# bcsefercik/markerless-robot-camera-calibration

Hardware: AMD Instinct MI355X
Metric: point-cloud frames/sec at 200k pts/frame (higher is better)
Workload: dtype f32

## Files before the change

### markerless-robot-camera-calibration_amd/csrc/sv_conv.hip

```cpp
#include <stdarg.h>
#include <stdio.h>
#include <stdlib.h>
#include <vector>

#include "sv_conv_params.h"

namespace sv {

static thread_local char g_last_instance[128] = "";
static thread_local double g_want_scale_override = -1.0;
static thread_local double g_tail_override = -1.0;
void note_instance(const char* fmt, ...) {
  va_list ap;
  va_start(ap, fmt);
  vsnprintf(g_last_instance, sizeof(g_last_instance), fmt, ap);
  va_end(ap);
}
#ifndef SV_CONV_WANT_SCALE_DEFAULT
#define SV_CONV_WANT_SCALE_DEFAULT 0.3
#endif
#ifndef SV_CONV_TAIL_DEFAULT
#define SV_CONV_TAIL_DEFAULT 0.15
#endif
constexpr int chunk_for(int tm, int waves_n) {
  if (waves_n == 1) return tm <= 64 ? 128 : 64;
  if (waves_n == 2) return tm <= 32 ? 128 : (tm <= 64 ? 64 : 32);
  return tm <= 16 ? 128 : (tm <= 32 ? 64 : 32);
}

constexpr int fused_offsets(int cpo) { return cpo == 0 ? 1 : (cpo < 8 ? 27 : (128 / cpo > 0 ? 128 / cpo : 1)); }
constexpr int lds_row_stride(int kc) {
  for (int sa = kc + 2;; ++sa)
    if (sa % 64 == 34 || (sa % 4 == 0 && (sa / 4) % 2 == 1)) return sa;
}

template <int TM_, int WAVES_N, int NT, int CPO = 0>
struct ConvCfg {
  static constexpr int WAVES_M = 4 / WAVES_N;
  static constexpr int MR = TM_ / WAVES_M / 16;
  static constexpr int TN = WAVES_N * NT * 16;
  static constexpr int GK = fused_offsets(CPO);
  static constexpr int KC = CPO ? (GK * CPO + 3) / 4 * 4 : chunk_for(TM_, WAVES_N);
  static constexpr int SA = lds_row_stride(KC);
  static constexpr int PFD_RAW = MR * NT >= 6 ? 1 : (8 + MR * NT - 1) / (MR * NT);
  static constexpr int PFD = PFD_RAW > KC / 4 ? KC / 4 : PFD_RAW;
  static constexpr bool USE_FULL = (MR * NT == 1) || (TM_ == 32 && WAVES_N == 4 && NT == 3) || (TM_ == 16 && NT == 3);
  static constexpr int F4_PER_ROW = KC / 4;
  static constexpr int ROWS_PER_PASS = 256 / F4_PER_ROW;
  static constexpr int A_F4 = (TM_ + ROWS_PER_PASS - 1) / ROWS_PER_PASS;
  static_assert(MR >= 1, "tile too small for the wave layout");
  static constexpr size_t lds_bytes(int K) { return (size_t)(2 * TM_ * SA + K * TM_) * sizeof(float); }
};

template <int TM_, int WAVES_N, int NT, bool FAST, int CPO = 0, bool RING = false, bool FULL = false>
__device__ __forceinline__ void conv_tile_body(const ConvParams& p, const int bidx, const int tile_base) {
  static_assert(FAST || !FULL, "FULL is a refinement of the FAST form");
  using Cfg = ConvCfg<TM_, WAVES_N, NT, CPO>;
  constexpr int MR = Cfg::MR, TN = Cfg::TN, A_F4 = Cfg::A_F4, KC = Cfg::KC, SA = Cfg::SA, GK = Cfg::GK;
  constexpr int PFD = RING ? Cfg::PFD : 1;
  constexpr int ROWS_PER_PASS = Cfg::ROWS_PER_PASS;
  constexpr int SUBS = TM_ / 16;
  extern __shared__ __attribute__((aligned(16))) float lds[];
  float* As = lds;
  int* idx_s = (int*)(lds + 2 * TM_ * SA);

  const int tid = threadIdx.x;
  const int lane = tid & 63;
  const int wid = __builtin_amdgcn_readfirstlane(tid >> 6);
  const int wm = wid / WAVES_N, wn = wid % WAVES_N;
  unsigned long long trace_t0 = 0, trace_t_loop = 0, trace_t_epi = 0;
  int trace_steps = 0;
  if (p.trace) trace_t0 = wall_clock64();
  const int ny = (p.Cout + TN - 1) / TN;
  constexpr int SUB_PER_PLAN_TILE = PLAN_TILE / TM_;
  const int t_lin = bidx / ny;
  const int t128 = tile_base + t_lin / SUB_PER_PLAN_TILE;
  const int p128 = p.tile_order ? p.tile_order[t128] : ((int)(p.Vpad / PLAN_TILE) - 1 - t128);
  const int tile = p128 * SUB_PER_PLAN_TILE + (t_lin % SUB_PER_PLAN_TILE);
  const int n0 = (bidx % ny) * TN;
  const int64_t row0 = (int64_t)tile * TM_;
  const int li = lane & 15, lq = lane >> 4;
  const int K = p.K, Cin = p.Cin, Cout = p.Cout;
  const int col0 = n0 + wn * NT * 16 + NT * li;
  const bool cols_full = col0 + NT <= Cout;

  f32x4 acc[MR][NT];
#pragma unroll
  for (int s = 0; s < MR; ++s)
#pragma unroll
    for (int n = 0; n < NT; ++n) acc[s][n] = (f32x4){0.f, 0.f, 0.f, 0.f};

  if (p.acc_init) {
    if constexpr (FAST) {
      const __amdgpu_buffer_rsrc_t rsrc_acc = __builtin_amdgcn_make_buffer_rsrc((void*)p.acc_init, 0, (int)p.acc_bytes, 0x00020000);
      int o_acc[MR][4];
      load_perm_rows<MR>(p, row0 + wm * MR * 16, lane >> 4, o_acc);
#pragma unroll
      for (int s = 0; s < MR; ++s)
#pragma unroll
        for (int reg = 0; reg < 4; ++reg) {
          const auto v = buffer_load_floats<NT>(
              rsrc_acc, o_acc[s][reg] >= 0 ? (uint32_t)o_acc[s][reg] * (uint32_t)(p.acc_ld * 4) + (uint32_t)col0 * 4u : BUF_ABSENT, 0u);
#pragma unroll
          for (int n = 0; n < NT; ++n) acc[s][n][reg] = v[n];
        }
    } else {
#pragma unroll
      for (int s = 0; s < MR; ++s)
#pragma unroll
        for (int reg = 0; reg < 4; ++reg) {
          const int64_t r = row0 + wm * MR * 16 + s * 16 + (lane >> 4) * 4 + reg;
          const int64_t o = p.perm ? (int64_t)p.perm[r] : (r < p.V_out ? r : -1);
#pragma unroll
          for (int n = 0; n < NT; ++n) acc[s][n][reg] = (o >= 0 && col0 + n < Cout) ? p.acc_init[o * p.acc_ld + col0 + n] : 0.0f;
        }
    }
  }
  uint32_t dense_mask = (1u << SUBS) - 1u;
  if (p.submask == nullptr) {
    const int64_t rem = p.V_out - row0;
    const int nsub = rem >= TM_ ? SUBS : (int)((rem + 15) / 16);
    dense_mask = (1u << nsub) - 1u;
  }
  if constexpr (FAST) {
    constexpr int STAGE_IT = (32 * TM_ + 255) / 256;
    int n_st[STAGE_IT];
#pragma unroll
    for (int it = 0; it < STAGE_IT; ++it) {
      const int e = tid + 256 * it;
      const int k = e / TM_, r = e % TM_;
      n_st[it] = -1;
      if (e < K * TM_) {
        if (p.nbr_s)
          n_st[it] = p.nbr_s[(int64_t)k * p.Vpad + row0 + r];
        else
          n_st[it] = (row0 + r < p.V_out) ? (int)(row0 + r) : -1;
      }
    }
#pragma unroll
    for (int it = 0; it < STAGE_IT; ++it) {
      const int e = tid + 256 * it;
      if (e < K * TM_) idx_s[e] = (int)(n_st[it] >= 0 ? (uint32_t)n_st[it] * (uint32_t)(p.in_ld * 4) : BUF_ABSENT);
    }
  } else {
    for (int e = tid; e < K * TM_; e += 256) {
      const int k = e / TM_, r = e - k * TM_;
      int n;
      if (p.nbr_s)
        n = p.nbr_s[(int64_t)k * p.Vpad + row0 + r];
      else
        n = (row0 + r < p.V_out) ? (int)(row0 + r) : -1;
      idx_s[e] = n;
    }
  }
  const __amdgpu_buffer_rsrc_t rsrc_in = __builtin_amdgcn_make_buffer_rsrc((void*)p.in, 0, (int)p.in_bytes, 0x00020000);
  const __amdgpu_buffer_rsrc_t rsrc_w = __builtin_amdgcn_make_buffer_rsrc((void*)p.W, 0, (int)p.w_bytes, 0x00020000);

  const int64_t sm_word = row0 / PLAN_TILE;
  const int sm_shift = (int)((row0 % PLAN_TILE) / 16);
  uint32_t my_sm = 0;
  if (lane < K) my_sm = p.submask ? ((p.submask[sm_word * K + lane] >> sm_shift) & ((1u << SUBS) - 1u)) : dense_mask;
  const uint32_t amask = (uint32_t)__ballot(my_sm != 0);
  auto fused_mask = [&](int k0) -> uint32_t {
    uint32_t m = 0;
#pragma unroll
    for (int g = 0; g < GK; ++g) m |= (uint32_t)__builtin_amdgcn_readlane((int)my_sm, min(k0 + g, 31));
    return m;
  };
  int k_n, c_n = 0;
  uint32_t sm_n = 0;
  bool have_n;
  if (CPO) {
    k_n = 0;
    while (k_n < K && (sm_n = fused_mask(k_n)) == 0) k_n += GK;
    have_n = k_n < K;
  } else {
    k_n = amask ? __builtin_ctz(amask) : K;
    sm_n = amask ? (uint32_t)__builtin_amdgcn_readlane((int)my_sm, k_n) : 0u;
    have_n = amask != 0;
  }
  auto advance = [&]() {
    if (CPO) {
      k_n += GK;
      while (k_n < K && (sm_n = fused_mask(k_n)) == 0) k_n += GK;
      have_n = k_n < K;
      return;
    }
    c_n += KC;
    if (c_n >= Cin) {
      c_n = 0;
      const uint32_t rest = amask & ~((2u << k_n) - 1u);
      have_n = rest != 0;
      k_n = have_n ? __builtin_ctz(rest) : K;
      sm_n = (uint32_t)__builtin_amdgcn_readlane((int)my_sm, have_n ? k_n : 0);
    }
  };

  float4 ra[A_F4];
  const int a_cc = (tid % Cfg::F4_PER_ROW) * 4;
  const int a_r = tid / Cfg::F4_PER_ROW;

  const uint32_t col_bytes = (uint32_t)a_cc * 4u;
  const int cin_rem = Cin % KC;
  const uint32_t col_last = (cin_rem == 0 || a_cc < cin_rem) ? col_bytes : 0u - (uint32_t)(Cin - cin_rem) * 4u;
  auto load_a = [&](int k, int c0, uint32_t sm) {
#pragma unroll
    for (int j = 0; j < A_F4; ++j) {
      const int r = a_r + ROWS_PER_PASS * j;
      if (FAST) {
        const int rr = (A_F4 * ROWS_PER_PASS > TM_) ? min(r, TM_ - 1) : r;
        if (CPO) {
          const int kk = k + a_cc / (CPO ? CPO : 1);
          uint32_t off = (uint32_t)idx_s[min(kk, K - 1) * TM_ + rr];
          if (kk >= K) off = BUF_ABSENT;
          const f32x4 v = buffer_load_floats<4>(rsrc_in, off + (uint32_t)(a_cc % (CPO ? CPO : 1)) * 4u, 0u);
          ra[j] = make_float4(v[0], v[1], v[2], v[3]);
        } else {
          const uint32_t off = (uint32_t)idx_s[k * TM_ + rr];
          const uint32_t cb = (!FULL && c0 + KC > Cin) ? col_last : col_bytes;
          const f32x4 v = buffer_load_floats<4>(rsrc_in, off + cb, (uint32_t)c0 * 4u);
          ra[j] = make_float4(v[0], v[1], v[2], v[3]);
        }
        (void)sm;
      } else if (CPO) {
        float e[4] = {0.f, 0.f, 0.f, 0.f};
        if (r < TM_ && ((sm >> (r >> 4)) & 1u)) {
#pragma unroll
          for (int q = 0; q < 4; ++q) {
            const int i = a_cc + q, kk = k + i / (CPO ? CPO : 1), c = i % (CPO ? CPO : 1);
            if (i < GK * CPO && kk < K) {
              const int n = idx_s[kk * TM_ + r];
              if (n >= 0) e[q] = p.in[(int64_t)n * p.in_ld + c];
            }
          }
        }
        ra[j] = make_float4(e[0], e[1], e[2], e[3]);
      } else {
        float4 v = make_float4(0.f, 0.f, 0.f, 0.f);
        if (r < TM_ && ((sm >> (r >> 4)) & 1u)) {
          const int n = idx_s[k * TM_ + r];
          const int c = c0 + a_cc;
          if (n >= 0) {
            const float* src = p.in + (int64_t)n * p.in_ld + c;
            if (p.vec_a) {
              if (c < Cin) v = *(const float4*)src;
            } else {
              if (c + 0 < Cin) v.x = src[0];
              if (c + 1 < Cin) v.y = src[1];
              if (c + 2 < Cin) v.z = src[2];
              if (c + 3 < Cin) v.w = src[3];
            }
          }
        }
        ra[j] = v;
      }
    }
  };
  auto store_a = [&](float* dstbuf, uint32_t sm) {
#pragma unroll
    for (int j = 0; j < A_F4; ++j) {
      const int r = a_r + ROWS_PER_PASS * j;
      if (r < TM_ && (FAST || ((sm >> (r >> 4)) & 1u))) {
        float2* dst = (float2*)(dstbuf + r * SA + a_cc);
        dst[0] = make_float2(ra[j].x, ra[j].y);
        dst[1] = make_float2(ra[j].z, ra[j].w);
      }
    }
  };

  typedef float bvec_t __attribute__((ext_vector_type(NT)));
  typedef float bvec_load_t __attribute__((ext_vector_type(NT), aligned(4)));
  bvec_t b[KC / 4];
  const int b_off = lq * Cout + col0;
  const uint32_t b_off_bytes = (uint32_t)b_off * 4u;
  auto step_weights = [&](int k, int c0) -> const float* { return p.W + ((int64_t)k * Cin + c0) * Cout; };
  auto cols_of = [&](int k, int c0) { return CPO ? min(GK, K - k) * CPO : min(KC, Cin - c0); };
  auto ksteps_of = [&](int k, int c0) { return (cols_of(k, c0) + 3) >> 2; };
  auto load_b = [&](const float* wstep, int k, int c0, int ksteps_valid, int ks, bvec_t& dst) {
    if (FAST) {
      const uint32_t row = (uint32_t)(k * Cin + c0 + (ks < ksteps_valid ? 4 * ks : 0));
      dst = buffer_load_floats<NT>(rsrc_w, b_off_bytes, row * (uint32_t)Cout * 4u);
      (void)wstep;
    } else {
      const int i = 4 * ks + lq;
      const float* src = p.W + ((int64_t)k * Cin + c0 + i) * Cout + col0;
      const bool row_ok = i < cols_of(k, c0);
#pragma unroll
      for (int n = 0; n < NT; ++n) dst[n] = (row_ok && col0 + n < Cout) ? src[n] : 0.0f;
    }
  };

  __syncthreads();
  if (have_n) {
    int k_c = k_n, c_c = c_n;
    uint32_t sm_c = sm_n;
    load_a(k_c, c_c, sm_c);
#pragma unroll
    for (int ks = 0; ks < KC / 4; ++ks) load_b(step_weights(k_c, c_c), k_c, c_c, ksteps_of(k_c, c_c), ks, b[ks]);
    store_a(As, sm_c);
    advance();
    int k_x = k_n, c_x = c_n;
    uint32_t sm_x = sm_n;
    bool have_x = have_n;
    __syncthreads();
    int buf = 0;
    if (p.trace) trace_t_loop = wall_clock64();

    auto step = [&]() -> bool {
      if (FAST || have_x) load_a(have_x ? k_x : 0, have_x ? c_x : 0, have_x ? sm_x : 0u);
      const float* a_base = As + buf * (TM_ * SA) + (wm * MR * 16 + li) * SA + lq;
      const uint32_t smw = (sm_c >> (wm * MR)) & ((1u << MR) - 1u);
      const int ksteps = ksteps_of(k_c, c_c);
      const int kb = have_x ? k_x : 0;
      const int cb = have_x ? c_x : 0;
      const float* wnext = step_weights(kb, cb);
      const int ksteps_next = ksteps_of(kb, cb);
      {
        auto reload_b = [&](int ks) {
          if (FULL) {
            b[ks] = buffer_load_floats<NT>(rsrc_w, b_off_bytes, (uint32_t)(kb * Cin + cb + 4 * ks) * (uint32_t)Cout * 4u);
          } else if (FAST || have_x) {
            load_b(wnext, kb, cb, ksteps_next, ks, b[ks]);
          }
        };
        auto mfma_row = [&](int ks, const float (&a)[MR]) {
#pragma unroll
          for (int s = 0; s < MR; ++s) {
            if ((MR == 1 && Cfg::WAVES_M == 1) || ((smw >> s) & 1u)) {
#pragma unroll
              for (int n = 0; n < NT; ++n)
                acc[s][n] = __builtin_amdgcn_mfma_f32_16x16x4f32(a[s], b[ks][n], acc[s][n], 0, 0, 0);
            }
          }
        };
        if constexpr (PFD == 1) {
          float a_cur[MR];
#pragma unroll
          for (int s = 0; s < MR; ++s) a_cur[s] = a_base[s * 16 * SA];
#pragma unroll
          for (int ks = 0; ks < KC / 4; ++ks) {
            if (FULL || ks < ksteps) {
              float a_nx[MR];
              if (ks + 1 < KC / 4) {
#pragma unroll
                for (int s = 0; s < MR; ++s) a_nx[s] = a_base[s * 16 * SA + (ks + 1) * 4];
                if (FULL) __builtin_amdgcn_sched_barrier(0);
              }
              mfma_row(ks, a_cur);
              if (ks + 1 < KC / 4) {
#pragma unroll
                for (int s = 0; s < MR; ++s) a_cur[s] = a_nx[s];
              }
            }
            reload_b(ks);
            if (FULL) __builtin_amdgcn_sched_barrier(0);
          }
        } else {
          float a_ring[PFD + 1][MR];
#pragma unroll
          for (int d = 0; d < PFD; ++d)
#pragma unroll
            for (int s = 0; s < MR; ++s) a_ring[d][s] = a_base[s * 16 * SA + d * 4];
#pragma unroll
          for (int ks = 0; ks < KC / 4; ++ks) {
            if (FULL || ks < ksteps) {
              if (ks + PFD < KC / 4) {
#pragma unroll
                for (int s = 0; s < MR; ++s)
                  a_ring[(ks + PFD) % (PFD + 1)][s] = a_base[s * 16 * SA + (ks + PFD) * 4];
                if (FULL) __builtin_amdgcn_sched_barrier(0);
              }
              mfma_row(ks, a_ring[ks % (PFD + 1)]);
            }
            reload_b(ks);
            if (FULL) __builtin_amdgcn_sched_barrier(0);
          }
        }
      }
      ++trace_steps;
      if (!have_x) return false;
      store_a(As + (buf ^ 1) * (TM_ * SA), sm_x);
      k_c = k_x;
      c_c = c_x;
      sm_c = sm_x;
      advance();
      k_x = k_n;
      c_x = c_n;
      sm_x = sm_n;
      have_x = have_n;
      __syncthreads();
      buf ^= 1;
      return true;
    };
    while (step()) {
    }
  }

  if (p.trace) trace_t_epi = wall_clock64();
  float sc[NT], sh[NT];
#pragma unroll
  for (int n = 0; n < NT; ++n) {
    const bool ok = col0 + n < Cout;
    sc[n] = (p.scale && ok) ? p.scale[col0 + n] : 1.0f;
    sh[n] = (p.shift && ok) ? p.shift[col0 + n] : 0.0f;
  }
  if constexpr (FAST) {
    epilogue_buffered<MR, NT>(p, acc, row0 + wm * MR * 16, lq, col0);
  } else
#pragma unroll
  for (int s = 0; s < MR; ++s) {
#pragma unroll
    for (int reg = 0; reg < 4; ++reg) {
      const int64_t r = row0 + wm * MR * 16 + s * 16 + lq * 4 + reg;
      int64_t o;
      if (p.perm)
        o = p.perm[r];
      else
        o = (r < p.V_out) ? r : -1;
      if (o < 0) continue;
      float y[NT];
#pragma unroll
      for (int n = 0; n < NT; ++n) {
        float v = acc[s][n][reg];
        if (p.scale)
          v = __builtin_fmaf(v, sc[n], sh[n]);
        else if (p.shift)
          v = v + sh[n];
        y[n] = v;
      }
      if (p.residual) {
        const float* res = p.residual + o * p.res_ld + col0;
#pragma unroll
        for (int n = 0; n < NT; ++n)
          if (col0 + n < Cout) y[n] = y[n] + res[n];
      }
      float* dst = p.out + o * p.out_ld + col0;
#pragma unroll
      for (int n = 0; n < NT; ++n) {
        float v = y[n];
        if (p.act == SV_ACT_RELU)
          v = v < 0.f ? 0.f : v;
        else if (p.act == SV_ACT_LEAKY_RELU)
          v = v > 0.f ? v : v * p.slope;
        if (col0 + n < Cout) dst[n] = v;
      }
    }
  }
  if (p.trace && tid == 0) {
    unsigned long long* t = p.trace + (size_t)blockIdx.x * 4;
    t[0] = trace_t0;
    t[1] = wall_clock64();
    t[2] = ((unsigned long long)__builtin_amdgcn_s_getreg((31 << 11) | 20) << 32) |
           (unsigned)__builtin_amdgcn_s_getreg((31 << 11) | 4);
    const unsigned long long pro = trace_t_loop ? ((trace_t_loop - trace_t0) >> 4) & 0xffffull : 0ull;
    const unsigned long long epi = ((t[1] - trace_t_epi) >> 4) & 0xffffull;
    t[3] = (unsigned long long)(unsigned)trace_steps | (pro << 32) | (epi << 48);
  }
}

template <int TM_, int WAVES_N, int NT, bool FAST, int CPO = 0, bool RING = false, bool FULL = false>
__global__ __launch_bounds__(256) void conv_fwd_kernel(ConvParams p) {
  conv_tile_body<TM_, WAVES_N, NT, FAST, CPO, RING, FULL>(p, (int)blockIdx.x, 0);
}

template <int TM_, int TAIL_TM, int WAVES_N, int NT, bool FAST>
__global__ __launch_bounds__(256) void conv_fwd_dual_kernel(ConvParams p) {
  if ((int)blockIdx.x < p.main_blocks)
    conv_tile_body<TM_, WAVES_N, NT, FAST>(p, (int)blockIdx.x, 0);
  else
    conv_tile_body<TAIL_TM, WAVES_N, NT, FAST>(p, (int)blockIdx.x - p.main_blocks, p.main_tiles128);
}

template <class Launch>
static int launch_traced(ConvParams& q, unsigned grid, int tm, int wn, int nt, hipStream_t stream, Launch&& launch) {
  static const char* trace_path = getenv("SV_CONV_TRACE");
  q.trace = nullptr;
  if (trace_path) SV_HIP(hipMalloc((void**)&q.trace, (size_t)grid * 4 * sizeof(unsigned long long)));
  launch();
  SV_LAUNCH_CHECK();
  if (q.trace) {
    std::vector<unsigned long long> host((size_t)grid * 4);
    SV_HIP(hipStreamSynchronize(stream));
    SV_HIP(hipMemcpy(host.data(), q.trace, host.size() * sizeof(unsigned long long), hipMemcpyDeviceToHost));
    SV_HIP(hipFree(q.trace));
    if (FILE* f = fopen(trace_path, "ab")) {
      const long long hdr[8] = {0x5356545243ll, (long long)grid, tm, wn, nt, q.ny, q.K, q.Cin};
      fwrite(hdr, sizeof(hdr), 1, f);
      fwrite(host.data(), sizeof(unsigned long long), host.size(), f);
      fclose(f);
    }
  }
  return SV_OK;
}

template <int TM_, int WAVES_N, int NT, int CPO = 0>
static int launch_conv(const ConvParams& p, hipStream_t stream) {
  using Cfg = ConvCfg<TM_, WAVES_N, NT, CPO>;
  ConvParams q = p;
  q.ntiles = (int)(p.Vpad / TM_);
  q.ny = (p.Cout + Cfg::TN - 1) / Cfg::TN;
  dim3 grid((unsigned)(q.ntiles * q.ny));
  const bool fast = p.vec_a && p.buf_ok && (p.Cout % Cfg::TN == 0);
  const bool ring = Cfg::PFD > 1 && grid.x <= 1024;
  constexpr bool F = (CPO % 4 == 0);
  const size_t lds = Cfg::lds_bytes(p.K);
  const bool full = Cfg::USE_FULL && (CPO ? (p.K % Cfg::GK == 0) : (p.Cin % Cfg::KC == 0));
  const int rc = launch_traced(q, grid.x, TM_, WAVES_N, NT, stream, [&] {
    if (F && fast && full) {
      if (ring)
        hipLaunchKernelGGL((conv_fwd_kernel<TM_, WAVES_N, NT, F, CPO, (Cfg::PFD > 1), (F && Cfg::USE_FULL)>), grid, dim3(256), lds, stream, q);
      else
        hipLaunchKernelGGL((conv_fwd_kernel<TM_, WAVES_N, NT, F, CPO, false, (F && Cfg::USE_FULL)>), grid, dim3(256), lds, stream, q);
    } else if (F && fast) {
      if (ring)
        hipLaunchKernelGGL((conv_fwd_kernel<TM_, WAVES_N, NT, F, CPO, (Cfg::PFD > 1)>), grid, dim3(256), lds, stream, q);
      else
        hipLaunchKernelGGL((conv_fwd_kernel<TM_, WAVES_N, NT, F, CPO, false>), grid, dim3(256), lds, stream, q);
    } else {
      if (ring)
        hipLaunchKernelGGL((conv_fwd_kernel<TM_, WAVES_N, NT, false, CPO, (Cfg::PFD > 1)>), grid, dim3(256), lds, stream, q);
      else
        hipLaunchKernelGGL((conv_fwd_kernel<TM_, WAVES_N, NT, false, CPO, false>), grid, dim3(256), lds, stream, q);
    }
  });
  if (rc != SV_OK) return rc;
  {
    const bool f = F && fast;
    if (CPO)
      note_instance("conv_fwd_kernel<%d, %d, %d, fused %d>|fast=%d,ring=%d,full=%d", TM_, WAVES_N, NT, CPO, (int)f, (int)ring,
                    (int)(f && full));
    else
      note_instance("conv_fwd_kernel<%d, %d, %d>|fast=%d,ring=%d,full=%d", TM_, WAVES_N, NT, (int)f, (int)ring, (int)(f && full));
  }
  return SV_OK;
}

template <int TM_, int TAIL_TM, int WAVES_N, int NT>
static int launch_conv_dual(const ConvParams& p, hipStream_t stream, double tail_fraction) {
  using Main = ConvCfg<TM_, WAVES_N, NT, 0>;
  using Tail = ConvCfg<TAIL_TM, WAVES_N, NT, 0>;
  const bool fast = p.vec_a && p.buf_ok && (p.Cout % Main::TN == 0);
  const int n128 = (int)(p.Vpad / PLAN_TILE);
  const int tail128 = (int)(n128 * tail_fraction);
  if (!fast || !p.tile_order || tail128 < 1 || tail128 >= n128) return SV_ERR_INVALID;
  ConvParams q = p;
  q.ny = p.Cout / Main::TN;
  q.main_tiles128 = n128 - tail128;
  q.main_blocks = q.main_tiles128 * (PLAN_TILE / TM_) * q.ny;
  q.ntiles = (int)(p.Vpad / TM_);
  const unsigned grid = (unsigned)(q.main_blocks + tail128 * (PLAN_TILE / TAIL_TM) * q.ny);
  const size_t lds = Main::lds_bytes(p.K) > Tail::lds_bytes(p.K) ? Main::lds_bytes(p.K) : Tail::lds_bytes(p.K);
  const int rc = launch_traced(q, grid, TM_, WAVES_N, NT, stream, [&] {
    hipLaunchKernelGGL((conv_fwd_dual_kernel<TM_, TAIL_TM, WAVES_N, NT, true>), dim3(grid), dim3(256), lds, stream, q);
  });
  if (rc != SV_OK) return rc;
  note_instance("conv_fwd_dual_kernel<%d, %d, %d, %d>|fast=1,ring=0,full=0", TM_, TAIL_TM, WAVES_N, NT);
  return SV_OK;
}

struct Candidate {
  int tm, wn, nt;
  int64_t want;
  int cpo;
};

template <int TM_, int WAVES_N, int NT, int CPO = 0>
static bool try_launch(const Candidate& c, const ConvParams& p, hipStream_t stream, int& rc) {
  if (c.tm == TM_ && c.wn == WAVES_N && c.nt == NT && c.cpo == CPO) {
    rc = launch_conv<TM_, WAVES_N, NT, CPO>(p, stream);
    return true;
  }
  return false;
}

static int launch_candidate(const Candidate& c, const ConvParams& p, hipStream_t stream) {
  int rc = SV_ERR_INVALID;
  if (try_launch<128, 4, 3>(c, p, stream, rc) || try_launch<128, 2, 3>(c, p, stream, rc) ||
      try_launch<128, 1, 3>(c, p, stream, rc) || try_launch<64, 4, 3>(c, p, stream, rc) ||
      try_launch<64, 2, 3>(c, p, stream, rc) || try_launch<64, 1, 3>(c, p, stream, rc) ||
      try_launch<32, 4, 3>(c, p, stream, rc) || try_launch<32, 2, 3>(c, p, stream, rc) ||
      try_launch<16, 4, 3>(c, p, stream, rc) ||
      try_launch<128, 4, 2>(c, p, stream, rc) || try_launch<128, 2, 2>(c, p, stream, rc) ||
      try_launch<128, 1, 2>(c, p, stream, rc) || try_launch<64, 4, 2>(c, p, stream, rc) ||
      try_launch<64, 2, 2>(c, p, stream, rc) || try_launch<64, 1, 2>(c, p, stream, rc) ||
      try_launch<32, 4, 2>(c, p, stream, rc) || try_launch<32, 2, 2>(c, p, stream, rc) ||
      try_launch<16, 4, 2>(c, p, stream, rc) ||
      try_launch<64, 4, 1>(c, p, stream, rc) || try_launch<32, 4, 1>(c, p, stream, rc) ||
      try_launch<16, 4, 1>(c, p, stream, rc) || try_launch<128, 2, 1>(c, p, stream, rc) ||
      try_launch<64, 2, 1>(c, p, stream, rc) || try_launch<32, 2, 1>(c, p, stream, rc) ||
      try_launch<128, 1, 1>(c, p, stream, rc) || try_launch<64, 1, 1>(c, p, stream, rc) ||
      try_launch<64, 2, 1, 3>(c, p, stream, rc) || try_launch<32, 2, 1, 3>(c, p, stream, rc) ||
      try_launch<64, 2, 1, 32>(c, p, stream, rc) || try_launch<32, 2, 1, 32>(c, p, stream, rc) ||
      try_launch<32, 4, 1, 32>(c, p, stream, rc) || try_launch<16, 4, 1, 32>(c, p, stream, rc) ||
      try_launch<32, 4, 1, 64>(c, p, stream, rc) || try_launch<16, 4, 1, 64>(c, p, stream, rc))
    return rc;
  set_error("sv_conv_fwd: no kernel instance <%d,%d,%d> cpo %d", c.tm, c.wn, c.nt, c.cpo);
  return SV_ERR_INVALID;
}

static int64_t candidate_wgs(const Candidate& c, const ConvParams& p) {
  const int tn = c.wn * c.nt * 16;
  return (p.Vpad / c.tm) * ((p.Cout + tn - 1) / tn);
}

static int select_and_launch(const ConvParams& p, hipStream_t stream) {
  static const Candidate wide3[] = {{64, 4, 3, 2500}, {32, 4, 3, 1500}, {32, 2, 3, 0}};
  static const Candidate wide3_128[] = {{64, 4, 3, 2500}, {64, 4, 2, 1200}, {32, 4, 3, 1200}, {16, 4, 3, 0}};
  static const Candidate wide3_128_full[] = {{64, 4, 3, 2500}, {32, 4, 3, 1200}, {16, 4, 3, 0}};
  static const Candidate wide2[] = {{128, 4, 2, 1300}, {64, 4, 2, 1500}, {32, 4, 2, 1500}, {32, 2, 2, 0}};
  static const Candidate wide2_64[] = {{128, 4, 2, 1300}, {64, 4, 2, 1500}, {32, 4, 2, 1500}, {16, 4, 1, 0}};
  static const Candidate c64[] = {{64, 4, 1, 1500}, {32, 4, 1, 1500}, {16, 4, 1, 0}};
  static const Candidate c32[] = {{128, 2, 1, 1500}, {64, 2, 1, 1500}, {32, 2, 1, 0}};
  static const Candidate c16[] = {{128, 1, 1, 600}, {64, 1, 1, 0}};
  const Candidate* list;
  int n;
  const int Cout = p.Cout;
  if (Cout > 128 && (Cout % 192 == 0 || Cout % 96 == 0 || Cout > 2048)) {
    if (Cout % 128 != 0) { list = wide3; n = 3; }
    else if (p.Cin % 128 == 0 && p.vec_a) { list = wide3_128_full; n = 3; }
    else { list = wide3_128; n = 4; }
  }
  else if (Cout > 64) { list = Cout % 64 == 0 ? wide2_64 : wide2; n = 4; }
  else if (Cout > 32) { list = c64; n = 3; }
  else if (Cout > 16) { list = c32; n = 3; }
  else { list = c16; n = 2; }
  static const Candidate f3[] = {{64, 2, 1, 3000, 3}, {32, 2, 1, 0, 3}};
  static const Candidate f32_32[] = {{64, 2, 1, 3000, 32}, {32, 2, 1, 0, 32}};
  static const Candidate f32_64[] = {{32, 4, 1, 1500, 32}, {16, 4, 1, 0, 32}};
  static const Candidate f64_64[] = {{32, 4, 1, 1500, 64}, {16, 4, 1, 0, 64}};
  if (p.K > 1) {
    if (p.Cin == 3 && Cout > 16 && Cout <= 32) { list = f3; n = 2; }
    else if (p.Cin == 32 && p.vec_a && Cout == 32) { list = f32_32; n = 2; }
    else if (p.Cin == 32 && p.vec_a && Cout == 64) { list = f32_64; n = 2; }
    else if (p.Cin == 64 && p.vec_a && (Cout == 64 || Cout == 128)) { list = f64_64; n = 2; }
  }
  if (const char* f = getenv("SV_CONV_FORCE_RANGE")) {
    long long vmin = 0, vmax = 0;
    int cout = 0;
    Candidate c = {0, 0, 0, 0, 0};
    if (sscanf(f, "%lld:%lld:%d:%d,%d,%d", &vmin, &vmax, &cout, &c.tm, &c.wn, &c.nt) == 6 && p.Vpad >= vmin && p.Vpad <= vmax &&
        p.Cout == cout && p.K > 1)
      return launch_candidate(c, p, stream);
  }
  if (const char* f = getenv("SV_CONV_FORCE_DENSE")) {
    long long vmin = 0;
    int cout = 0;
    Candidate c = {0, 0, 0, 0, 0};
    if (sscanf(f, "%lld:%d:%d,%d,%d", &vmin, &cout, &c.tm, &c.wn, &c.nt) == 5 && p.Vpad >= vmin && p.Cout == cout && p.K == 1)
      return launch_candidate(c, p, stream);
  }
  if (const char* f = getenv("SV_CONV_FORCE")) {
    Candidate c = {0, 0, 0, 0, 0};
    if (sscanf(f, "%d,%d,%d,%d", &c.tm, &c.wn, &c.nt, &c.cpo) >= 3) return launch_candidate(c, p, stream);
  }
  static const double want_scale =
      getenv("SV_CONV_WANT_SCALE") ? atof(getenv("SV_CONV_WANT_SCALE")) : SV_CONV_WANT_SCALE_DEFAULT;
  static const double tail_fraction = getenv("SV_CONV_TAIL") ? atof(getenv("SV_CONV_TAIL")) : SV_CONV_TAIL_DEFAULT;
  const double ws = g_want_scale_override >= 0.0 ? g_want_scale_override : want_scale;
  const double tf = g_tail_override >= 0.0 ? g_tail_override : tail_fraction;
  for (int i = 0; i < n; ++i)
    if ((double)candidate_wgs(list[i], p) >= ws * (double)list[i].want) {
      const Candidate& c = list[i];
      if (c.tm == 64 && c.wn == 4 && c.nt == 3 && c.cpo == 0 && tf > 0.0 &&
          launch_conv_dual<64, 32, 4, 3>(p, stream, tf) == SV_OK)
        return SV_OK;
      return launch_candidate(c, p, stream);
    }
  return launch_candidate(list[n - 1], p, stream);
}

}

using namespace sv;

extern "C" const char* sv_conv_last_instance(void) { return sv::g_last_instance; }

extern "C" int sv_conv_set_dispatch(double want_scale, double tail_fraction) {
  SV_CHECK_ARG(tail_fraction < 1.0, "tail_fraction must be below 1");
  sv::g_want_scale_override = want_scale;
  sv::g_tail_override = tail_fraction;
  return SV_OK;
}

extern "C" int sv_conv_fwd(const float* in, int64_t V_in, int64_t in_ld, int Cin, const float* W, int K, int Cout,
                           const int32_t* perm, const int32_t* nbr_s, const uint32_t* submask,
                           const int32_t* tile_order, int64_t V_out, int64_t Vpad, const float* scale, const float* shift, const float* residual, int64_t res_ld,
                           int act, float slope, float* out, int64_t out_ld, sv_stream_t stream_) {
  return sv_conv_fwd_acc(in, V_in, in_ld, Cin, W, K, Cout, perm, nbr_s, submask, tile_order, V_out, Vpad, nullptr, 0, scale, shift,
                         residual, res_ld, act, slope, out, out_ld, stream_);
}

extern "C" int sv_conv_fwd_acc(const float* in, int64_t V_in, int64_t in_ld, int Cin, const float* W, int K, int Cout,
                               const int32_t* perm, const int32_t* nbr_s, const uint32_t* submask, const int32_t* tile_order,
                               int64_t V_out, int64_t Vpad, const float* acc_init, int64_t acc_ld, const float* scale,
                               const float* shift, const float* residual, int64_t res_ld, int act, float slope, float* out,
                               int64_t out_ld, sv_stream_t stream_) {
  hipStream_t stream = (hipStream_t)stream_;
  SV_CHECK_ARG(!acc_init || acc_ld >= Cout, "acc_init stride too small");
  SV_CHECK_ARG(Cin > 0 && Cout > 0 && K >= 1 && K <= 32, "bad channel / kernel volume");
  SV_CHECK_ARG(V_out >= 0 && Vpad >= V_out && Vpad % PLAN_TILE == 0, "Vpad must be a multiple of 128 >= V_out");
  SV_CHECK_ARG(in_ld >= Cin && out_ld >= Cout, "row strides too small");
  SV_CHECK_ARG(act >= SV_ACT_NONE && act <= SV_ACT_LEAKY_RELU, "bad activation");
  if (V_out == 0) return SV_OK;
  SV_CHECK_ARG(in && W && out, "null pointer");
  SV_CHECK_ARG(V_in >= 1, "V_in = rows of `in` (every index of the plan is below it)");
  const bool has_plan = perm || nbr_s || submask;
  SV_CHECK_ARG(!has_plan || (perm && nbr_s && submask), "perm, nbr_s and submask must be given together");
  SV_CHECK_ARG(has_plan || K == 1, "K > 1 needs a plan");
  SV_CHECK_ARG(!residual || res_ld >= Cout, "residual stride too small");
  ConvParams p;
  p.in = in; p.in_ld = in_ld; p.Cin = Cin; p.W = W; p.K = K; p.Cout = Cout;
  p.perm = perm; p.nbr_s = nbr_s; p.submask = submask; p.tile_order = tile_order; p.V_out = V_out; p.Vpad = Vpad;
  p.scale = scale; p.shift = shift; p.residual = residual; p.res_ld = res_ld;
  p.acc_init = acc_init; p.acc_ld = acc_ld;
  p.act = act; p.slope = slope; p.out = out; p.out_ld = out_ld;
  p.vec_a = (in_ld % 4 == 0) && (Cin % 4 == 0) && (((uintptr_t)in & 15) == 0);
  const uint64_t in_bytes = ((uint64_t)(V_in - 1) * (uint64_t)in_ld + (uint64_t)Cin) * 4u;
  const uint64_t w_bytes = (uint64_t)K * (uint64_t)Cin * (uint64_t)Cout * 4u;
  const uint64_t out_bytes = ((uint64_t)(V_out - 1) * (uint64_t)out_ld + (uint64_t)Cout) * 4u;
  const uint64_t res_bytes = residual ? ((uint64_t)(V_out - 1) * (uint64_t)res_ld + (uint64_t)Cout) * 4u : 0u;
  const uint64_t acc_bytes = acc_init ? ((uint64_t)(V_out - 1) * (uint64_t)acc_ld + (uint64_t)Cout) * 4u : 0u;
  p.buf_ok = in_bytes < BUF_LIMIT && w_bytes < BUF_LIMIT && out_bytes < BUF_LIMIT && res_bytes < BUF_LIMIT &&
             acc_bytes < BUF_LIMIT && (((uintptr_t)perm & 15) == 0);
  p.acc_bytes = p.buf_ok ? (uint32_t)acc_bytes : 0u;
  if (!p.buf_ok && !has_plan && K == 1 && w_bytes < BUF_LIMIT) {
    int64_t ld_max = in_ld > out_ld ? in_ld : out_ld;
    if (residual && res_ld > ld_max) ld_max = res_ld;
    const int64_t rows = (int64_t)((BUF_LIMIT - 4096u) / ((uint64_t)ld_max * 4u)) / PLAN_TILE * PLAN_TILE;
    if (rows >= PLAN_TILE && rows < V_out) {
      for (int64_t r0 = 0; r0 < V_out; r0 += rows) {
        const int64_t n = V_out - r0 < rows ? V_out - r0 : rows;
        const int rc = sv_conv_fwd_acc(in + r0 * in_ld, n, in_ld, Cin, W, K, Cout, nullptr, nullptr, nullptr, nullptr, n,
                                       (n + PLAN_TILE - 1) / PLAN_TILE * PLAN_TILE, acc_init ? acc_init + r0 * acc_ld : nullptr,
                                       acc_ld, scale, shift, residual ? residual + r0 * res_ld : nullptr, res_ld, act, slope,
                                       out + r0 * out_ld, out_ld, stream_);
        if (rc != SV_OK) return rc;
      }
      return SV_OK;
    }
  }
  p.in_bytes = p.buf_ok ? (uint32_t)in_bytes : 0u;
  p.w_bytes = p.buf_ok ? (uint32_t)w_bytes : 0u;
  p.out_bytes = p.buf_ok ? (uint32_t)out_bytes : 0u;
  p.res_bytes = p.buf_ok ? (uint32_t)res_bytes : 0u;
  p.ntiles = 0;
  p.ny = 0;
  p.trace = nullptr;
  p.main_blocks = 0;
  p.main_tiles128 = 0;
  if (has_plan && K > 1 && K <= 27 && Cin == 3 && Cout == 32 && !acc_init) {
    if (p.buf_ok) return launch_conv_first_mfma(p, stream);
    return launch_conv_first_layer(p, stream);
  }
  if (has_plan && K > 1 && K <= 32 && Cin == 32 && Cout == 32 && p.vec_a && p.buf_ok && !acc_init)
    return launch_conv_thin(p, stream, sv::g_want_scale_override >= 1.0);
  if (!has_plan && K == 1 && Cout <= 4 && p.vec_a && Cin >= 64 && !acc_init) return launch_linear_narrow(p, stream);
  return select_and_launch(p, stream);
}
```

Measured before the change: 73.88.

## Add wide software-pipelined step with rolling weight ring and split A gathers

Adds a specialised main-loop step for the FAST, non-ring, 4-wave, NT=3 configurations with 64- or 32-row tiles. It keeps a 4-deep rolling ring of weight registers that prefetches ahead into the next step's weights. It splits the next tile's A gathers into two halves, issued and written to LDS partway through the MFMA loop. A waves-per-EU hint of 5 is added for the TM=64 variant to steer register allocation and occupancy. The aim is to hide gather and weight-load latency behind MFMA work and cut register pressure from holding every k-step of B. The cost is more template specialisation and a risk of spills or a poorer schedule.

```diff
diff --git a/markerless-robot-camera-calibration_amd/csrc/sv_conv.hip b/markerless-robot-camera-calibration_amd/csrc/sv_conv.hip
--- a/markerless-robot-camera-calibration_amd/csrc/sv_conv.hip
+++ b/markerless-robot-camera-calibration_amd/csrc/sv_conv.hip
@@ -60,6 +60,8 @@
   constexpr int PFD = RING ? Cfg::PFD : 1;
   constexpr int ROWS_PER_PASS = Cfg::ROWS_PER_PASS;
   constexpr int SUBS = TM_ / 16;
+  constexpr bool WIDE = FAST && !FULL && !RING && CPO == 0 && WAVES_N == 4 && NT == 3 && (TM_ == 64 || TM_ == 32);
+  static_assert(!WIDE || A_F4 == 2, "the WIDE step moves a step's gathers in two halves");
   extern __shared__ __attribute__((aligned(16))) float lds[];
   float* As = lds;
   int* idx_s = (int*)(lds + 2 * TM_ * SA);
@@ -203,74 +205,78 @@
   const uint32_t col_bytes = (uint32_t)a_cc * 4u;
   const int cin_rem = Cin % KC;
   const uint32_t col_last = (cin_rem == 0 || a_cc < cin_rem) ? col_bytes : 0u - (uint32_t)(Cin - cin_rem) * 4u;
-  auto load_a = [&](int k, int c0, uint32_t sm) {
-#pragma unroll
-    for (int j = 0; j < A_F4; ++j) {
-      const int r = a_r + ROWS_PER_PASS * j;
-      if (FAST) {
-        const int rr = (A_F4 * ROWS_PER_PASS > TM_) ? min(r, TM_ - 1) : r;
-        if (CPO) {
-          const int kk = k + a_cc / (CPO ? CPO : 1);
-          uint32_t off = (uint32_t)idx_s[min(kk, K - 1) * TM_ + rr];
-          if (kk >= K) off = BUF_ABSENT;
-          const f32x4 v = buffer_load_floats<4>(rsrc_in, off + (uint32_t)(a_cc % (CPO ? CPO : 1)) * 4u, 0u);
-          ra[j] = make_float4(v[0], v[1], v[2], v[3]);
-        } else {
-          const uint32_t off = (uint32_t)idx_s[k * TM_ + rr];
-          const uint32_t cb = (!FULL && c0 + KC > Cin) ? col_last : col_bytes;
-          const f32x4 v = buffer_load_floats<4>(rsrc_in, off + cb, (uint32_t)c0 * 4u);
-          ra[j] = make_float4(v[0], v[1], v[2], v[3]);
-        }
-        (void)sm;
-      } else if (CPO) {
-        float e[4] = {0.f, 0.f, 0.f, 0.f};
-        if (r < TM_ && ((sm >> (r >> 4)) & 1u)) {
-#pragma unroll
-          for (int q = 0; q < 4; ++q) {
-            const int i = a_cc + q, kk = k + i / (CPO ? CPO : 1), c = i % (CPO ? CPO : 1);
-            if (i < GK * CPO && kk < K) {
-              const int n = idx_s[kk * TM_ + r];
-              if (n >= 0) e[q] = p.in[(int64_t)n * p.in_ld + c];
-            }
+  auto gather_row = [&](int k, int c0, uint32_t sm, int j) -> float4 {
+    const int r = a_r + ROWS_PER_PASS * j;
+    if (FAST) {
+      const int rr = (A_F4 * ROWS_PER_PASS > TM_) ? min(r, TM_ - 1) : r;
+      if (CPO) {
+        const int kk = k + a_cc / (CPO ? CPO : 1);
+        uint32_t off = (uint32_t)idx_s[min(kk, K - 1) * TM_ + rr];
+        if (kk >= K) off = BUF_ABSENT;
+        const f32x4 v = buffer_load_floats<4>(rsrc_in, off + (uint32_t)(a_cc % (CPO ? CPO : 1)) * 4u, 0u);
+        return make_float4(v[0], v[1], v[2], v[3]);
+      } else {
+        const uint32_t off = (uint32_t)idx_s[k * TM_ + rr];
+        const uint32_t cb = (!FULL && c0 + KC > Cin) ? col_last : col_bytes;
+        const f32x4 v = buffer_load_floats<4>(rsrc_in, off + cb, (uint32_t)c0 * 4u);
+        return make_float4(v[0], v[1], v[2], v[3]);
+      }
+      (void)sm;
+    } else if (CPO) {
+      float e[4] = {0.f, 0.f, 0.f, 0.f};
+      if (r < TM_ && ((sm >> (r >> 4)) & 1u)) {
+#pragma unroll
+        for (int q = 0; q < 4; ++q) {
+          const int i = a_cc + q, kk = k + i / (CPO ? CPO : 1), c = i % (CPO ? CPO : 1);
+          if (i < GK * CPO && kk < K) {
+            const int n = idx_s[kk * TM_ + r];
+            if (n >= 0) e[q] = p.in[(int64_t)n * p.in_ld + c];
           }
         }
-        ra[j] = make_float4(e[0], e[1], e[2], e[3]);
-      } else {
-        float4 v = make_float4(0.f, 0.f, 0.f, 0.f);
-        if (r < TM_ && ((sm >> (r >> 4)) & 1u)) {
-          const int n = idx_s[k * TM_ + r];
-          const int c = c0 + a_cc;
-          if (n >= 0) {
-            const float* src = p.in + (int64_t)n * p.in_ld + c;
-            if (p.vec_a) {
-              if (c < Cin) v = *(const float4*)src;
-            } else {
-              if (c + 0 < Cin) v.x = src[0];
-              if (c + 1 < Cin) v.y = src[1];
-              if (c + 2 < Cin) v.z = src[2];
-              if (c + 3 < Cin) v.w = src[3];
-            }
+      }
+      return make_float4(e[0], e[1], e[2], e[3]);
+    } else {
+      float4 v = make_float4(0.f, 0.f, 0.f, 0.f);
+      if (r < TM_ && ((sm >> (r >> 4)) & 1u)) {
+        const int n = idx_s[k * TM_ + r];
+        const int c = c0 + a_cc;
+        if (n >= 0) {
+          const float* src = p.in + (int64_t)n * p.in_ld + c;
+          if (p.vec_a) {
+            if (c < Cin) v = *(const float4*)src;
+          } else {
+            if (c + 0 < Cin) v.x = src[0];
+            if (c + 1 < Cin) v.y = src[1];
+            if (c + 2 < Cin) v.z = src[2];
+            if (c + 3 < Cin) v.w = src[3];
           }
         }
-        ra[j] = v;
-      }
+      }
+      return v;
+    }
+  };
+  auto load_a = [&](int k, int c0, uint32_t sm) {
+#pragma unroll
+    for (int j = 0; j < A_F4; ++j) ra[j] = gather_row(k, c0, sm, j);
+  };
+  auto scatter_row = [&](float* dstbuf, uint32_t sm, int j, const float4& v) {
+    const int r = a_r + ROWS_PER_PASS * j;
+    if (r < TM_ && (FAST || ((sm >> (r >> 4)) & 1u))) {
+      float2* dst = (float2*)(dstbuf + r * SA + a_cc);
+      dst[0] = make_float2(v.x, v.y);
+      dst[1] = make_float2(v.z, v.w);
     }
   };
   auto store_a = [&](float* dstbuf, uint32_t sm) {
 #pragma unroll
-    for (int j = 0; j < A_F4; ++j) {
-      const int r = a_r + ROWS_PER_PASS * j;
-      if (r < TM_ && (FAST || ((sm >> (r >> 4)) & 1u))) {
-        float2* dst = (float2*)(dstbuf + r * SA + a_cc);
-        dst[0] = make_float2(ra[j].x, ra[j].y);
-        dst[1] = make_float2(ra[j].z, ra[j].w);
-      }
-    }
+    for (int j = 0; j < A_F4; ++j) scatter_row(dstbuf, sm, j, ra[j]);
   };
 
   typedef float bvec_t __attribute__((ext_vector_type(NT)));
   typedef float bvec_load_t __attribute__((ext_vector_type(NT), aligned(4)));
-  bvec_t b[KC / 4];
+  constexpr int KS = KC / 4;
+  constexpr int BR = WIDE ? 4 : KS;
+  bvec_t b[BR];
   const int b_off = lq * Cout + col0;
   const uint32_t b_off_bytes = (uint32_t)b_off * 4u;
   auto step_weights = [&](int k, int c0) -> const float* { return p.W + ((int64_t)k * Cin + c0) * Cout; };
@@ -296,7 +302,7 @@
     uint32_t sm_c = sm_n;
     load_a(k_c, c_c, sm_c);
 #pragma unroll
-    for (int ks = 0; ks < KC / 4; ++ks) load_b(step_weights(k_c, c_c), k_c, c_c, ksteps_of(k_c, c_c), ks, b[ks]);
+    for (int ks = 0; ks < BR; ++ks) load_b(step_weights(k_c, c_c), k_c, c_c, ksteps_of(k_c, c_c), ks, b[ks]);
     store_a(As, sm_c);
     advance();
     int k_x = k_n, c_x = c_n;
@@ -392,7 +398,71 @@
       buf ^= 1;
       return true;
     };
-    while (step()) {
+    auto step_wide = [&]() -> bool {
+      const int kb = have_x ? k_x : 0;
+      const int cb = have_x ? c_x : 0;
+      float* const a_next = As + (buf ^ 1) * (TM_ * SA);
+      ra[0] = gather_row(kb, cb, 0u, 0);
+      const float* a_base = As + buf * (TM_ * SA) + (wm * MR * 16 + li) * SA + lq;
+      const uint32_t smw = (sm_c >> (wm * MR)) & ((1u << MR) - 1u);
+      const int ksteps = ksteps_of(k_c, c_c);
+      const int ksteps_next = ksteps_of(kb, cb);
+      const uint32_t wrow_c = (uint32_t)(k_c * Cin + c_c);
+      const uint32_t wrow_x = (uint32_t)(kb * Cin + cb);
+      float a_cur[MR];
+#pragma unroll
+      for (int s = 0; s < MR; ++s) a_cur[s] = a_base[s * 16 * SA];
+#pragma unroll
+      for (int ks = 0; ks < KS; ++ks) {
+        if (ks < ksteps) {
+          float a_nx[MR];
+          if (ks + 1 < KS) {
+#pragma unroll
+            for (int s = 0; s < MR; ++s) a_nx[s] = a_base[s * 16 * SA + (ks + 1) * 4];
+          }
+#pragma unroll
+          for (int s = 0; s < MR; ++s) {
+            if ((smw >> s) & 1u) {
+#pragma unroll
+              for (int n = 0; n < NT; ++n)
+                acc[s][n] = __builtin_amdgcn_mfma_f32_16x16x4f32(a_cur[s], b[ks % BR][n], acc[s][n], 0, 0, 0);
+            }
+          }
+          if (ks + 1 < KS) {
+#pragma unroll
+            for (int s = 0; s < MR; ++s) a_cur[s] = a_nx[s];
+          }
+        }
+        const int kn = ks + BR < KS ? ks + BR : ks + BR - KS;
+        const uint32_t wrow = ks + BR < KS ? wrow_c + (uint32_t)(kn < ksteps ? 4 * kn : 0)
+                                           : wrow_x + (uint32_t)(kn < ksteps_next ? 4 * kn : 0);
+        b[ks % BR] = buffer_load_floats<NT>(rsrc_w, b_off_bytes, wrow * (uint32_t)Cout * 4u);
+        if (ks == KS / 2 - 1) {
+          scatter_row(a_next, 0u, 0, ra[0]);
+          ra[0] = gather_row(kb, cb, 0u, 1);
+        }
+      }
+      ++trace_steps;
+      if (!have_x) return false;
+      scatter_row(a_next, 0u, 1, ra[0]);
+      k_c = k_x;
+      c_c = c_x;
+      sm_c = sm_x;
+      advance();
+      k_x = k_n;
+      c_x = c_n;
+      sm_x = sm_n;
+      have_x = have_n;
+      __syncthreads();
+      buf ^= 1;
+      return true;
+    };
+    if constexpr (WIDE) {
+      while (step_wide()) {
+      }
+    } else {
+      while (step()) {
+      }
     }
   }
 
@@ -458,13 +528,19 @@
   }
 }
 
+constexpr unsigned wide_waves(int tm, int waves_n, int nt, bool fast, int cpo, bool ring, bool full) {
+  return (tm == 64 && waves_n == 4 && nt == 3 && fast && cpo == 0 && !ring && !full) ? 5u : 1u;
+}
+
 template <int TM_, int WAVES_N, int NT, bool FAST, int CPO = 0, bool RING = false, bool FULL = false>
-__global__ __launch_bounds__(256) void conv_fwd_kernel(ConvParams p) {
+__global__ __launch_bounds__(256) __attribute__((amdgpu_waves_per_eu(wide_waves(TM_, WAVES_N, NT, FAST, CPO, RING, FULL))))
+void conv_fwd_kernel(ConvParams p) {
   conv_tile_body<TM_, WAVES_N, NT, FAST, CPO, RING, FULL>(p, (int)blockIdx.x, 0);
 }
 
 template <int TM_, int TAIL_TM, int WAVES_N, int NT, bool FAST>
-__global__ __launch_bounds__(256) void conv_fwd_dual_kernel(ConvParams p) {
+__global__ __launch_bounds__(256) __attribute__((amdgpu_waves_per_eu(wide_waves(TM_, WAVES_N, NT, FAST, 0, false, false))))
+void conv_fwd_dual_kernel(ConvParams p) {
   if ((int)blockIdx.x < p.main_blocks)
     conv_tile_body<TM_, WAVES_N, NT, FAST>(p, (int)blockIdx.x, 0);
   else
```

After: 74.93, median of 6. 1.4% higher.
